# Prayforhanluo/HiCHap_master

Measured on AMD Instinct MI355X. Metric: ICE iterations/sec on 10 kb whole-genome matrix (also nnz*iters/sec), higher is better.
Workload: dtype f64; 1 GPU; hg19-10kb-diploid-wholegenome; n_bins=607282, nnz_upper=4998527599, resolution_bp=10000, parallelism=single GPU, entries_stored=9997055198, slots_u32=160483740, slots_u16=3356357472, payload_bytes=14884946704, tiles=89023, units=89007, hbm_bytes_matrix=15833045375

## Files before the change

hichap_master_amd/_lib.py:

```python
from __future__ import annotations

import ctypes as C
import os

_HERE = os.path.dirname(os.path.abspath(__file__))
LIB_PATH = os.environ.get("HH_LIB") or os.path.join(_HERE, "libhichap_hip.so")

HH_OK = 0


class HipLibraryError(RuntimeError):

    def __init__(self, code, msg):
        super().__init__(f"[hh rc={code}] {msg}")
        self.code = code


class MatrixInfo(C.Structure):
    _fields_ = [(n, C.c_int64) for n in (
        "n_bins", "row_lo", "row_hi", "nnz_upper", "n_entries", "n_slots", "n_tiles",
        "n_units", "n_wide", "device_bytes", "n_slots_narrow", "payload_bytes")] + [
        (n, C.c_int32) for n in ("n_chroms", "ignore_diags", "cis_only", "device", "band_w", "n_units_flat")] + [
        ("n_band", C.c_int64), ("payload_bytes_flat", C.c_int64)] + [
        (n, C.c_int32) for n in ("band_w4", "upper")]
# ... 7 lines not shown
        ("comp_block", C.c_int32), ("ignore_diags", C.c_int32), ("cis_only", C.c_int32),
        ("pad_", C.c_int32), ("seed", C.c_uint64)]


class IceOpts(C.Structure):
    _fields_ = [
        ("mad_max", C.c_int32), ("min_nnz", C.c_int32), ("min_count", C.c_double),
        ("tol", C.c_double), ("max_iters", C.c_int32), ("rescale_marginals", C.c_int32),
        ("check_every", C.c_int32), ("pad_", C.c_int32)]


P = C.c_void_p
I32, I64, F64 = C.c_int32, C.c_int64, C.c_double
PI32, PI64, PF64 = C.POINTER(C.c_int32), C.POINTER(C.c_int64), C.POINTER(C.c_double)

SIGNATURES = {
    "hh_last_error": (C.c_char_p, []),
    "hh_version": (C.c_int, []),
    "hh_device_count": (C.c_int, [PI32]),
    "hh_set_device": (C.c_int, [I32]),
    "hh_synchronize": (C.c_int, [P]),
    "hh_device_copy": (C.c_int, [P, P, I64, P]),
    "hh_tune": (C.c_int, [C.c_char_p, I64]),
    "hh_tune_get": (C.c_int, [C.c_char_p, PI64]),
    "hh_ktime_enable": (C.c_int, [I32]),
    "hh_ktime_query": (C.c_int, [C.c_char_p, P, P]),
    "hh_ktime_reset": (C.c_int, []),
    "hh_matrix_from_pixels": (C.c_int, [P, P, P, I64, I64, P, I32, I32, I32, I64, I64, P, C.POINTER(P)]),
    "hh_matrix_from_pixels_device": (C.c_int, [P, P, P, I64, I64, P, I32, I32, I32, I64, I64, P, C.POINTER(P)]),
    "hh_matrix_free": (C.c_int, [P]),
    "hh_matrix_get_info": (C.c_int, [P, C.POINTER(MatrixInfo)]),
    "hh_matrix_export_upper": (C.c_int, [P, P, P, P, PI64]),
    "hh_synth_count": (C.c_int, [C.POINTER(SynthParams), P, P, P]),
    "hh_synth_build": (C.c_int, [C.POINTER(SynthParams), I64, I64, P, C.POINTER(P)]),
    "hh_synth_dense": (C.c_int, [P, I32, P, P]),
    "hh_synth_pixels": (C.c_int, [C.POINTER(SynthParams), I32, P, C.POINTER(P)]),
    "hh_pixels_get": (C.c_int, [P, P, P, P, PI64]),
    "hh_pixels_free": (C.c_int, [P]),
    "hh_ice_balance": (C.c_int, [P, C.POINTER(IceOpts), P, P, P, P, P, PF64, P]),
    "hh_ice_create": (C.c_int, [P, C.POINTER(IceOpts), C.POINTER(P)]),
    "hh_ice_free": (C.c_int, [P]),
    "hh_ice_n_groups": (C.c_int, [P, PI32]),
    "hh_ice_marg_local": (C.c_int, [P, I32, P, P]),
    "hh_ice_set_marg": (C.c_int, [P, P, I32, I64, P, P]),
    "hh_ice_filter_nnz": (C.c_int, [P, P]),
    "hh_ice_filter_count_mad": (C.c_int, [P, P]),
    "hh_ice_update": (C.c_int, [P, P]),
    "hh_ice_active_groups": (C.c_int, [P, PI32, P]),
    "hh_ice_iterations_done": (C.c_int, [P, PI32]),
    "hh_ice_run": (C.c_int, [P, I32, P]),
    "hh_ice_finalize": (C.c_int, [P, P, P, P, P, P, P]),
    "hh_ice_last_sweep_timing": (C.c_int, [P, PF64, PI32, PF64]),
    "hh_ice_swept_bytes": (C.c_int, [P, PI64]),
    "hh_ice_get_bias": (C.c_int, [P, P, P]),
    "hh_ice_set_bias": (C.c_int, [P, P, P]),
    "hh_ice_uband_fallbacks": (C.c_int, [P, PI64, P]),
    "hh_ice_uband_skipped": (C.c_int, [P, PI64, PI64]),
    "hh_sweep_trace": (C.c_int, [P, I64, PI64]),
    "hh_matrix_stream_probe": (C.c_int, [P, I32, PF64, I32]),
    "hh_comm_unique_id": (C.c_int, [P]),
    "hh_comm_init": (C.c_int, [P, I32, I32, C.POINTER(P)]),
    "hh_comm_free": (C.c_int, [P]),
    "hh_comm_allgather": (C.c_int, [P, I64, P, P, P]),
    "hh_comm_reduce_scatter": (C.c_int, [P, I64, P, P, P]),
    "hh_ice_set_column_exchange": (C.c_int, [P, I32, I32, P, P, P, P, P]),
    "hh_ice_balance_sharded": (C.c_int, [P, C.POINTER(IceOpts), I32, I32, P, P, P, P, P, P, P, P, PF64, P]),
    "hh_ice_balance_cis_local": (C.c_int, [P, C.POINTER(IceOpts), I32, I64, P, P, P, P, P, P, P, PF64, P]),
    "hh_ice_filters_sharded": (C.c_int, [P, I32, P, P, P, P]),
    "hh_ice_run_sharded": (C.c_int, [P, I32, P, P, P, I32, P]),
    "hh_dense_rowstats": (C.c_int, [P, I32, I64, P, P, P, P, I32, P]),
    "hh_dense_symvc": (C.c_int, [P, I32, I64, P, P, F64, F64, P, I32, P]),
    "hh_twostep": (C.c_int, [P, P, P, I64, P, P, P, P, I32, P]),
    "hh_twostep_batch": (C.c_int, [I32, P, P, P, P, P, P, P, P, I32, P]),
    "hh_dense_from_cells": (C.c_int, [P, P, P, I64, I64, I64, I32, I32, P, P]),
    "hh_dense_upper_count": (C.c_int, [P, I64, PI64, P]),
    "hh_dense_upper_write": (C.c_int, [P, I64, P, P, P, P]),
    "hh_comp_create": (C.c_int, [P, I64, I32, P, C.POINTER(P)]),
    "hh_comp_free": (C.c_int, [P]),
    "hh_comp_colnnz": (C.c_int, [P, P, P]),
    "hh_comp_diag_sums": (C.c_int, [P, P, P, P]),
    "hh_comp_sliding_oe": (C.c_int, [P, P, I32, P]),
    "hh_comp_get_sliding_oe": (C.c_int, [P, P, P]),
    "hh_comp_correlation": (C.c_int, [P, P, P, I64, P]),
    "hh_comp_get_cor": (C.c_int, [P, P, P]),
    "hh_comp_set_cor": (C.c_int, [P, P, P]),
    "hh_gap_scan": (C.c_int, [P, I64, I32, I32, P, I32, P]),
    "hh_di_scan": (C.c_int, [P, I64, I32, P, P, I32, P, I32, P]),
    "hh_band_from_pixels": (C.c_int, [P, P, P, I64, P, I64, I64, I64, I32, P, I32, P]),
    "hh_tad_scan_pixels": (C.c_int, [P, P, P, I64, P, I64, I64, I64, I32, P, I32, P, P, I32, P]),
    "hh_insulation_scan": (C.c_int, [P, I64, I32, P, P, I32, I32, P, P, I32, P]),
    "hh_insulation_pixels": (C.c_int, [P, P, P, I64, P, I64, I64, I64, P, P, I32, I32, P, P, I32, P]),
    "hh_viterbi_gmm": (C.c_int, [P, I64, I32, I32, P, P, P, P, P, P, P]),
    "hh_hmm_bw_create": (C.c_int, [P, P, I64, I32, I32, P, C.POINTER(P)]),
    "hh_hmm_bw_free": (C.c_int, [P]),
    "hh_hmm_bw_step": (C.c_int, [P, P, P, P, P, P, F64, PF64]),
    "hh_hmm_bw_train": (C.c_int, [P, P, P, P, P, P, I32, F64, F64, PI32, P, PI32]),
    "hh_hmm_bw_last_step_ms": (C.c_int, [P, PF64]),
    "hh_comp_pca": (C.c_int, [P, I32, F64, I32, P, P, P, P]),
    "hh_comp_select_stats": (C.c_int, [P, P, I32, F64, P, P]),
    "hh_comp_pca_status": (C.c_int, [P, PI32, PI32, PI32, PI32]),
    "hh_sym_topk": (C.c_int, [P, I32, I32, P, P]),
    "hh_binner_create": (C.c_int, [I32, C.c_char_p, P, I32, I32, C.POINTER(P)]),
    "hh_binner_free": (C.c_int, [P]),
    "hh_binner_add_target": (C.c_int, [P, I32, I32, P, P, I64, PI32]),
    "hh_binner_feed": (C.c_int, [P, C.c_char_p, I64, P, I64, P]),
    "hh_binner_add_impute_target": (C.c_int, [P, I32, I32, P, P, I64, P, I32, I64, F64, PI32]),
# ... 130 lines not shown
```

hichap_master_amd/csrc/ice.hip:

```cpp
#include <algorithm>
#include <chrono>
#include <functional>
#include <cmath>
#include <limits>

#include "ice_internal.hpp"

namespace hh {
constexpr int kThreads = 256;

constexpr int kSweepThreads = 512;
constexpr int kSweepWaves = kSweepThreads / 64;
constexpr int kFlatU = 8;
static_assert(kFlatU == kFlatIlvU, "k_sweep_flatw walks the interleaved layout's runs");

__device__ __forceinline__ double lds_b(const double* bl, uint32_t byteoff) {
    return *reinterpret_cast<const double*>(reinterpret_cast<const char*>(bl) + byteoff);
}

__device__ __forceinline__ void tile_dot(const uint4 v, const double* __restrict__ bl, double& a0, double& a1) {
    const uint32_t w[4] = {v.x, v.y, v.z, v.w};
    double x[4];
#pragma unroll
    for (int i = 0; i < 4; ++i) x[i] = lds_b(bl, w[i] & 0xFFFFu);
// ... 2314 lines not shown

using namespace hh;

namespace hh {
constexpr int kFuseMaxTiles = 128;
}

struct hh_ice {
    hh_matrix* m = nullptr;
    hh_ice_opts o{};
    int64_t n = 0, nloc = 0;
    int32_t G = 1;
    std::vector<int64_t> glo, ghi;
    int32_t n_tiles = 0;
    DBuf<int32_t> tile_lo, tile_hi, tile_group, group_tile_ptr, blk_tile_ptr;
    DBuf<double> bias, marg, part, tile_cnt, tile_sum, tile_sq, g_cnt, g_sum;
    DBuf<unsigned> counter;
    bool stats_fresh = false;
    DBuf<double> bpart;
    int32_t nch = 0;
    int32_t nchu = 0;
    DBuf<double> upart;
    DBuf<uint32_t> ub_tasks[2];
    int64_t ub_ntasks[2] = {0, 0}, ub_bytes[2] = {0, 0}, ub_waves_all = 0, ub_waves_dead = 0;
    DBuf<unsigned long long> ub_fallbacks;
    DBuf<uint8_t> halo8, halo4;
    int64_t halo_lo = 0, ub_glo = 0, ub_ghi = 0;
    DBuf<uint8_t> active;
    DBuf<double> g_var, g_mean;
    DBuf<int32_t> g_iters;
    DBuf<uint8_t> g_empty;
    DBuf<long long> rank_rows;
    std::vector<int64_t> h_rank_rows;
    DBuf<unsigned long long> colpart, colacc, bmax, bfix;
    DBuf<double> fix;
    double rmax = 1.0;
    bool rmax_global = false;
    int32_t cx_world = 1, cx_rank = 0;
    int64_t cx_maxlen = 0;
    std::vector<int64_t> cx_rr;
    DBuf<long long> cx_rr_dev;
    hh_reduce_fn cx_fn = nullptr;
    void* cx_user = nullptr;
    hh_allgather_fn cx_ag = nullptr;
    void* cx_ag_user = nullptr;
    DBuf<unsigned long long> cx_send, cx_recv, cx_all;
    int32_t iters_done = 0;
    PinnedBuf<uint8_t> h_active;
    std::vector<hipEvent_t> ev;
    double sweep_ms = 0.0, iter_ms = 0.0;
    int32_t sweep_launches = 0;
    hipStream_t side = nullptr, side2 = nullptr;
    hipEvent_t fork = nullptr, join = nullptr, join2 = nullptr;
    ~hh_ice() {
        for (auto e : ev) (void)hipEventDestroy(e);
        if (join2) (void)hipEventDestroy(join2);
        if (side2) (void)hipStreamDestroy(side2);
        if (fork) (void)hipEventDestroy(fork);
        if (join) (void)hipEventDestroy(join);
        if (side) (void)hipStreamDestroy(side);
    }
    bool full() const { return m->row_lo == 0 && m->row_hi == m->n_bins; }
    TileArgs ta() {
        return TileArgs{tile_lo.p, tile_hi.p, tile_group.p, group_tile_ptr.p, blk_tile_ptr.p, tile_cnt.p,
                        tile_sum.p, tile_sq.p, g_cnt.p, g_sum.p, counter.p};
    }
    bool small_stats() const { return hh::g_fuse_stats == 1 || (hh::g_fuse_stats < 0 && n_tiles <= hh::kFuseMaxTiles); }
    uint8_t* act() { return active.p + (iters_done & 1) * G; }
    uint8_t* nxt() { return active.p + (1 - (iters_done & 1)) * G; }
};

namespace hh {

constexpr int64_t kConcUbMinBytes = 1LL << 30;
constexpr int64_t kUbandMinBytes = 128LL << 20;
constexpr int64_t kSingleMaxBytes = 1LL << 30;

using FlatwKernel = void (*)(TileDev, const uint8_t*, const double*, long long, double*);
template <int PIPE>
static FlatwKernel flatw_by_waves(int nw) {
    switch (nw) {
        case 8: return k_sweep_flatw<kFlatU, PIPE, 8, false>;
        case 10: return k_sweep_flatw<kFlatU, PIPE, 10, false>;
        case 11: return k_sweep_flatw<kFlatU, PIPE, 11, false>;
    }
    return nullptr;
}
static FlatwKernel flatw_kernel(int pipe, int nw) {
    switch (pipe) {
        case 0: return flatw_by_waves<0>(nw);
        case 2: return flatw_by_waves<2>(nw);
        case 3: return flatw_by_waves<3>(nw);
    }
    return nullptr;
}

template <bool UP>
static void launch_sweep(const hh_matrix* m, const TileDev& T, const uint8_t* act, const double* b, double* part,
                            hipStream_t s, hipStream_t s_tiled, int which) {
    const int n_tiled = (int)(m->n_units - m->n_units_flat), n_flat = (int)m->n_units_flat;
    auto tiled = [&] {
        if (!n_tiled) return;
        HH_KTIME("k_sweep_tiled", s_tiled);
        auto kern = k_sweep_tiled<UP, 0>;
        if constexpr (!UP) {
            if (g_tiled_pf == 1) kern = k_sweep_tiled<UP, 1>;
            if (g_tiled_pf == 2) kern = k_sweep_tiled<UP, 2>;
        }
// ... 209 lines not shown
                    : rows == 128 ? k_sweep_bands<128, true>
                                  : k_sweep_bands<256, false>;
        hipLaunchKernelGGL(kern, dim3(rb, (unsigned)nc), dim3(kBandThreads), 0, s, L, (long long)S->nloc,
                           (long long)m->row_lo, (long long)m->n_bins, S->act(), m->row_group.p, S->bias.p,
                           S->bpart.p);
        HIP_CHECK(hipGetLastError());
    };
    if (g_band_fused) {
        launch(segs, ch);
    } else {
        for (int k = 0; k < segs.n; ++k) {
            BandSegs one{};
            one.s[0] = segs.s[k];
            one.n = 1;
            for (int y = 0; y < segs.s[k].nc; ++y) one.ord[y] = (uint8_t)(segs.s[k].ch + y);
            launch(one, segs.s[k].nc);
        }
    }
}

static void sweep_single(hh_ice* S, hipStream_t s) {
    const hh_matrix* m = S->m;
    BandSegs segs;
    const int ch = (S->nch && S->nloc && !S->nchu) ? band_segs(m, segs) : (segs = BandSegs{}, 0);
    const int band_rb = (int)((S->nloc + 63) / 64);
    const int n_tiled = (int)(m->n_units - m->n_units_flat), n_flat = (int)m->n_units_flat;
    const long long n_band = ch ? (long long)band_rb * ch : 0;
    const long long grid = n_tiled + n_band + n_flat;
    if (S->nchu && S->nloc) sweep_uband(S, s);
    if (!grid) return;
    HH_REQUIRE(grid < (1LL << 31), "sweep grid too large for one launch");
    unsigned long long* trace = grid <= g_trace_cap ? g_trace : nullptr;
    if (trace) g_trace_n = grid;
    auto kern = k_sweep_all<kFlatU, false>;
    if constexpr (kUpperBuild) {
        if (m->upper && S->colpart.p) kern = k_sweep_all<kFlatU, true>;
    }
    hipLaunchKernelGGL(kern, dim3((unsigned)grid), dim3(kSweepThreads), 0, s, tdev(S), S->act(), n_tiled,
                       (int)n_band, segs, band_rb, (long long)S->nloc, (long long)m->row_lo, m->row_group.p,
                       S->bias.p, (long long)m->n_bins, S->part.p, S->bpart.p, trace);
    HIP_CHECK(hipGetLastError());
}

static void ensure_side_streams(hh_ice* S) {
    if (S->side) return;
    int cur = 0;
    HIP_CHECK(hipGetDevice(&cur));
    if (cur != S->m->device) HIP_CHECK(hipSetDevice(S->m->device));
    HIP_CHECK(hipStreamCreateWithFlags(&S->side, hipStreamNonBlocking));
    HIP_CHECK(hipEventCreateWithFlags(&S->fork, hipEventDisableTiming));
    HIP_CHECK(hipEventCreateWithFlags(&S->join, hipEventDisableTiming));
    HIP_CHECK(hipStreamCreateWithFlags(&S->side2, hipStreamNonBlocking));
    HIP_CHECK(hipEventCreateWithFlags(&S->join2, hipEventDisableTiming));
    if (cur != S->m->device) HIP_CHECK(hipSetDevice(cur));
}

static void marg_weighted(hh_ice* S, double* out, hipStream_t s, bool timed, int slot) {
    hh_matrix* m = S->m;
    const bool up = m->upper && S->colpart.p;
    const bool shard_x = up && S->cx_world > 1;
    HH_REQUIRE(!shard_x || S->rmax_global,
               "upper-triangle tiles on a shard: run the filters on the gathered marginals first (global scale)");
    if (timed) HIP_CHECK(hipEventRecord(S->ev[2 * slot], s));
    if (up)
        hipLaunchKernelGGL(k_fixscale, dim3(nblocks(std::max<int64_t>(S->n, 1), 256)), dim3(256), 0, s, S->bmax.p,
                           S->iters_done & 1, S->rmax, S->fix.p, S->bias.p, (long long)S->n, S->bfix.p);
    const TileDev T = tdev(S);
    {
        HH_KTIME(timed ? nullptr : "ice_sweep", s);
        const int64_t bytes = 4 * m->n_slots + 2 * m->n_slots_narrow + (int64_t)m->band.n + (int64_t)m->band4.n;
        const bool conc = g_band_concurrent && (S->nch || S->nchu) && S->nloc && m->n_units &&
                          (bytes >= g_conc_min_bytes || (S->nchu && bytes >= kConcUbMinBytes));
        const bool single = !(up && m->n_fgroups) && !m->flat_perm &&
                            (g_sweep_single == 1 || (g_sweep_single == -1 && bytes < kSingleMaxBytes));
        if (single) {
            sweep_single(S, s);
        } else if (conc) {
            ensure_side_streams(S);
            HIP_CHECK(hipEventRecord(S->fork, s));
            HIP_CHECK(hipStreamWaitEvent(S->side, S->fork, 0));
            if (g_split_tiles) HIP_CHECK(hipStreamWaitEvent(S->side2, S->fork, 0));
            if (g_conc_order == 1) {
                sweep(m, T, S->act(), S->bias.p, S->part.p, s, s, 2);
                sweep_band(S, S->side);
                sweep(m, T, S->act(), S->bias.p, S->part.p, s, g_split_tiles ? S->side2 : s, 1);
            } else if (g_conc_order == 2) {
                sweep(m, T, S->act(), S->bias.p, S->part.p, s, s, 2);
                sweep(m, T, S->act(), S->bias.p, S->part.p, s, g_split_tiles ? S->side2 : s, 1);
                sweep_band(S, S->side);
            } else {
                sweep_band(S, S->side);
                sweep(m, T, S->act(), S->bias.p, S->part.p, s, g_split_tiles ? S->side2 : s);
            }
            HIP_CHECK(hipEventRecord(S->join, S->side));
            if (g_split_tiles) {
                HIP_CHECK(hipEventRecord(S->join2, S->side2));
                HIP_CHECK(hipStreamWaitEvent(s, S->join2, 0));
            }
            HIP_CHECK(hipStreamWaitEvent(s, S->join, 0));
        } else {
            sweep(m, T, S->act(), S->bias.p, S->part.p, s);
            sweep_band(S, s);
        }
        if (up && S->n > 0) {
            hipLaunchKernelGGL(k_colsum, dim3(nblocks(S->n, 256)), dim3(256), 0, s, S->colpart.p, m->jslot_ptr.p,
                               m->jslot.p, 0LL, (long long)S->n, S->colacc.p);
            HIP_CHECK(hipGetLastError());
        }
    }
    if (timed) HIP_CHECK(hipEventRecord(S->ev[2 * slot + 1], s));
    const unsigned long long* col_own = up ? S->colacc.p + m->row_lo : nullptr;
    if (shard_x) {
        const long long tot = (long long)S->cx_world * S->cx_maxlen;
        hipLaunchKernelGGL(k_colpad, dim3(nblocks(tot, kThreads)), dim3(kThreads), 0, s, S->colacc.p, S->cx_world,
                           (long long)S->cx_maxlen, S->cx_rr_dev.p, S->cx_send.p);
        HIP_CHECK(hipGetLastError());
        int rc = 0;
        if (S->cx_fn) {
            rc = S->cx_fn(reinterpret_cast<const int64_t*>(S->cx_send.p), S->cx_maxlen,
                          reinterpret_cast<int64_t*>(S->cx_recv.p), S->cx_user, s);
        } else {
            rc = S->cx_ag(reinterpret_cast<const double*>(S->cx_send.p), tot, reinterpret_cast<double*>(S->cx_all.p),
                          S->cx_ag_user, s);
            if (!rc)
                hipLaunchKernelGGL(k_colgather, dim3(nblocks(S->cx_maxlen, kThreads)), dim3(kThreads), 0, s,
                                   S->cx_all.p, S->cx_world, (long long)S->cx_maxlen, S->cx_rank, S->cx_recv.p);
        }
        if (rc) HH_THROW(rc < 0 ? rc : HH_ERR_HIP, std::string("column exchange failed: ") + hh_last_error());
        col_own = S->cx_recv.p;
    }
// ... 47 lines not shown
}

}

static void filter_count_mad(hh_ice* S, hipStream_t s,
                             const std::function<std::vector<double>(const std::vector<double>&)>& gather) {
    if (S->o.min_count != 0.0)
        hipLaunchKernelGGL(k_filter_lt, dim3(nblocks(S->n, kThreads)), dim3(kThreads), 0, s, S->marg.p,
                           (long long)S->n, S->o.min_count, S->bias.p);
    HIP_CHECK(hipGetLastError());
    if (S->o.mad_max <= 0) return;
    std::vector<double> marg(S->n), bias(S->n);
    {
        PinnedDown dl;
        dl.add(S->marg.p, marg.data(), (size_t)S->n);
        dl.add(S->bias.p, bias.data(), (size_t)S->n);
        dl.run(s);
    }
    const auto& off = S->m->chrom_offsets;
    std::vector<double> pos;
    for (int c = 0; c < S->m->n_chroms; ++c) {
        pos.clear();
        for (int64_t i = off[c]; i < off[c + 1]; ++i)
            if (marg[i] > 0) pos.push_back(marg[i]);
        const double med = np_median(pos);
        for (int64_t i = off[c]; i < off[c + 1]; ++i) marg[i] = marg[i] / med;
    }
    const std::vector<double> all = gather ? gather(marg) : marg;
    std::vector<double> logm;
    for (double x : all)
        if (x > 0) logm.push_back(std::log(x));
    const double med = np_median(logm);
    std::vector<double> dev(logm.size());
    for (size_t k = 0; k < logm.size(); ++k) dev[k] = std::fabs(logm[k] - med);
    const double cutoff = std::exp(med - S->o.mad_max * np_median(dev));
    for (int64_t i = 0; i < S->n; ++i)
        if (marg[i] < cutoff) bias[i] = 0.0;
    upload_pinned_sync(S->bias.p, bias.data(), (size_t)S->n, s);
}

extern "C" {

int hh_ice_create(hh_matrix* m, const hh_ice_opts* o, hh_ice** out) {
    return guard([&] {
        HH_REQUIRE(m && out, "null");
        check_opts(o);
        HIP_CHECK(hipSetDevice(m->device));
        auto S = std::make_unique<hh_ice>();
        S->m = m;
        S->o = *o;
        if (S->o.check_every <= 0) S->o.check_every = 8;
        S->n = m->n_bins;
        S->nloc = m->nloc();
        if (m->cis_only) {
            S->G = m->n_chroms;
            for (int c = 0; c < m->n_chroms; ++c) {
                S->glo.push_back(m->chrom_offsets[c]);
                S->ghi.push_back(m->chrom_offsets[c + 1]);
            }
        } else {
            S->G = 1;
            S->glo = {0};
            S->ghi = {m->n_bins};
        }
        std::vector<int32_t> tlo, thi, tg, gtp(S->G + 1, 0);
        for (int g = 0; g < S->G; ++g) {
            gtp[g] = (int32_t)tlo.size();
            for (int64_t b = S->glo[g]; b < S->ghi[g];) {
                const int64_t e = std::min<int64_t>((b / kR + 1) * kR, S->ghi[g]);
                tlo.push_back((int32_t)b);
                thi.push_back((int32_t)e);
                tg.push_back(g);
                b = e;
            }
        }
        gtp[S->G] = (int32_t)tlo.size();
        S->n_tiles = (int32_t)tlo.size();
        const int64_t nblk = (S->n + kR - 1) / kR;
        std::vector<int32_t> btp(nblk + 1, 0);
        for (size_t t = 0, B = 0; B <= (size_t)nblk; ++B) {
            while (t < tlo.size() && tlo[t] < (int64_t)B * kR) ++t;
            btp[B] = (int32_t)t;
        }
        hipStream_t s = 0;
        S->tile_lo = to_device(tlo, s);
        S->tile_hi = to_device(thi, s);
        S->tile_group = to_device(tg, s);
        S->group_tile_ptr = to_device(gtp, s);
        S->blk_tile_ptr = to_device(btp, s);
        S->g_cnt.alloc(S->G);
        S->g_sum.alloc(S->G);
        S->counter.alloc(2);
        S->counter.zero(s);
        S->bias.alloc(S->n);
        std::vector<double> ones(S->n, 1.0);
        upload_pinned_sync(S->bias.p, ones.data(), (size_t)S->n, s);
        S->marg.alloc(S->n);
        S->marg.zero(s);
        S->part.alloc(std::max<int64_t>(m->n_part, 1));
        S->nch = m->band_w > 0 ? (int32_t)((band_stride(m->band_w) + kBandChunk - 1) / kBandChunk) : 0;
        if (m->band_w4 > m->band_w)
            S->nch += 2 * (int32_t)((band4_seg(m->band_w, m->band_w4) + kBandChunk - 1) / kBandChunk);
        const int64_t band_all = m->n_bins * ((m->band_w > 0 ? band_stride(m->band_w) : 0) +
                                              (m->band_w4 > m->band_w ? band4_stride(m->band_w, m->band_w4) : 0));
        if (S->nch && (g_uband == 2 || (g_uband == 1 && band_all >= kUbandMinBytes))) {
            const long long dmax = std::max<long long>(m->band_w, m->band_w4);
// ... 160 lines not shown
        hipStream_t s = as_stream(stream);
        HIP_CHECK(hipMemcpyAsync(S->h_active.p, S->act(), S->G, hipMemcpyDeviceToHost, s));
        HIP_CHECK(hipStreamSynchronize(s));
        int a = 0;
        for (int g = 0; g < S->G; ++g) a += S->h_active.p[g] ? 1 : 0;
        *n_active = a;
    });
}

int hh_ice_iterations_done(const hh_ice* S, int32_t* iters) {
    return guard([&] { HH_REQUIRE(S && iters, "null"); *iters = S->iters_done; });
}

int hh_ice_run(hh_ice* S, int32_t n, void* stream) {
    return guard([&] {
        HH_REQUIRE(S && n >= 0, "bad arguments");
        HH_REQUIRE(S->full(), "hh_ice_run needs a matrix holding every row (use the sharded API)");
        hipStream_t s = as_stream(stream);
        const size_t need = 2 * (size_t)n + 2;
        while (S->ev.size() < need) {
            hipEvent_t e;
            HIP_CHECK(hipEventCreate(&e));
            S->ev.push_back(e);
        }
        HIP_CHECK(hipEventRecord(S->ev[2 * n], s));
        const bool ev = g_iter_events != 0;
        for (int k = 0; k < n; ++k) {
            marg_weighted(S, S->marg.p, s, ev, k);
            update(S, s);
        }
        HIP_CHECK(hipEventRecord(S->ev[2 * n + 1], s));
        HIP_CHECK(hipStreamSynchronize(s));
        double tot = 0.0;
        for (int k = 0; ev && k < n; ++k) {
            float ms = 0.f;
            HIP_CHECK(hipEventElapsedTime(&ms, S->ev[2 * k], S->ev[2 * k + 1]));
            tot += ms;
        }
        float all = 0.f;
        HIP_CHECK(hipEventElapsedTime(&all, S->ev[2 * n], S->ev[2 * n + 1]));
        S->sweep_ms = tot;
        S->iter_ms = all;
        S->sweep_launches = n;
    });
}

int hh_ice_last_sweep_timing(const hh_ice* S, double* sweep_ms_total, int32_t* sweep_launches,
                             double* iter_ms_total) {
    return guard([&] {
        HH_REQUIRE(S, "null");
        if (sweep_ms_total) *sweep_ms_total = S->sweep_ms;
        if (sweep_launches) *sweep_launches = S->sweep_launches;
        if (iter_ms_total) *iter_ms_total = S->iter_ms;
    });
}

int hh_ice_set_column_exchange(hh_ice* S, int32_t world, int32_t rank, const int64_t* rank_rows, hh_reduce_fn reduce,
                               void* reduce_user, hh_allgather_fn allgather, void* allgather_user) {
    return guard([&] {
        HH_REQUIRE(S && world >= 1 && rank_rows && rank >= -1 && rank < world, "bad arguments");
        HH_REQUIRE(world == 1 || reduce || allgather || (S->cx_fn && S->cx_world == world),
                   "a reduce or all-gather function is required for world > 1");
        std::vector<int64_t> rr(rank_rows, rank_rows + world + 1);
        HH_REQUIRE(rr[0] == 0 && rr[world] == S->n, "rank_rows must span [0, n_bins]");
        int64_t maxlen = 1;
        for (int k = 0; k < world; ++k) {
            HH_REQUIRE(rr[k] <= rr[k + 1], "rank_rows not monotone");
            maxlen = std::max<int64_t>(maxlen, rr[k + 1] - rr[k]);
        }
        if (rank < 0) {
            for (int k = 0; k < world && rank < 0; ++k)
                if (rr[k] == S->m->row_lo && rr[k + 1] == S->m->row_hi) rank = k;
            HH_REQUIRE(rank >= 0, "the matrix shard is none of rank_rows' ranges");
        }
        HH_REQUIRE(rr[rank] == S->m->row_lo && rr[rank + 1] == S->m->row_hi,
                   "the matrix shard does not hold rank_rows[rank] .. rank_rows[rank + 1]");
        if (!reduce && S->cx_fn && S->cx_world == world) {
            reduce = S->cx_fn;
            reduce_user = S->cx_user;
        }
        S->cx_world = world;
        S->cx_rank = rank;
        S->cx_maxlen = maxlen;
        S->cx_fn = reduce;
        S->cx_user = reduce_user;
        S->cx_ag = allgather;
        S->cx_ag_user = allgather_user;
        if (rr != S->cx_rr) {
            S->cx_rr = rr;
            std::vector<long long> ll(rr.begin(), rr.end());
            S->cx_rr_dev = to_device(ll, 0);
            HIP_CHECK(hipStreamSynchronize(0));
        }
        if (world > 1 && S->m->upper) {
            S->cx_send.alloc((size_t)world * maxlen);
            S->cx_recv.alloc((size_t)maxlen);
            if (!reduce) S->cx_all.alloc((size_t)world * world * maxlen);
        }
    });
}

int hh_ice_get_bias(const hh_ice* S, double* bias, void* stream) {
    return guard([&] {
        HH_REQUIRE(S && bias, "null");
        hipStream_t s = as_stream(stream);
        S->bias.download(bias, S->n, s);
// ... 276 lines not shown
```

hichap_master_amd/csrc/ice_internal.hpp:

```cpp
#pragma once

#include "hh_common.hpp"

namespace hh {

constexpr int kR = 512;
#ifndef HH_KWBITS
#define HH_KWBITS 13
#endif
constexpr int kWBits = HH_KWBITS;
constexpr bool kUpperBuild = HH_KWBITS <= 12;
constexpr int kW = 1 << kWBits;
constexpr uint32_t kColMask = kW - 1;
constexpr uint32_t kCntMax = 65535u;
inline int64_t g_unit_entries = 0;
constexpr int64_t kMaxBins = (int64_t)1 << 30;

constexpr uint32_t kNarrowMax = 7;

constexpr int kBandChunk = 2048;
constexpr int kBandMaxW = 16384;
constexpr uint32_t kBandMaxCnt = 255u;
constexpr double kBandDensity = 0.5;
inline int64_t g_band_w = -1;
// ... 193 lines not shown
    }
    hh::TileDev dev(unsigned long long* colpart = nullptr, const double* fix = nullptr,
                    const unsigned long long* bfix = nullptr) const {
        return hh::TileDev{pay.p, payn.p, tile_J.p, tile_ent.p, tile_rp.p, tile_entn.p, tile_rpn.p, u_tlo.p,
                           u_thi.p, u_rb.p, u_rlo.p, u_rhi.p, u_slot.p, u_glo.p, u_ghi.p, blk_unit_ptr.p,
                           u_order.p, tile_perm.p, tile_band.p, tile_fw.p, tile_frec.p,
                           reinterpret_cast<const uint4*>(frec.p), u_whole.p, fg_ptr.p, fg_unit.p, fg_desc.p,
                           hh::g_flat_defer, upper && colpart ? 1 : 0, (long long)row_lo, u_cslot.p, fg_cslot.p,
                           colpart, fix, bfix};
    }
};

namespace hh {
inline std::vector<uint16_t> bin_groups(const hh_matrix& m) {
    std::vector<uint16_t> g(m.n_bins, 0);
    if (m.cis_only)
        for (int c = 0; c < m.n_chroms; ++c)
            for (int64_t b = m.chrom_offsets[c]; b < m.chrom_offsets[c + 1]; ++b) g[b] = (uint16_t)c;
    return g;
}
void upload_plan(const TilePlan& P, hh_matrix& m, hipStream_t s);

constexpr int kFlatIlvU = 8;
__host__ __device__ inline uint32_t flat_ilv_cnt(uint32_t m, int k) {
    return m > (uint32_t)k ? (m - (uint32_t)k + kFlatIlvU - 1) / kFlatIlvU : 0u;
}
__host__ __device__ inline uint32_t flat_ilv_pos(uint32_t m, uint32_t i) {
    const int k = (int)(i % kFlatIlvU);
    uint32_t b = 0;
    for (int j = 0; j < k; ++j) b += flat_ilv_cnt(m, j);
    return b + i / kFlatIlvU;
}
void finalize_flat_layout(hh_matrix& m, hipStream_t s);
void narrow_payload_plain(const hh_matrix& m, DBuf<uint16_t>& out, hipStream_t s);
void dev_sort_u64(DBuf<unsigned long long>& keys, int64_t n, int bits, hipStream_t s, int lo_bit = 0);
int64_t dev_sort_cells_by_col(const int32_t* r, const int32_t* c, const uint32_t* v, int64_t nnz, int fmt, int ib,
                              int cbits, DBuf<unsigned long long>& keys, hipStream_t s);
void dev_excl_scan_i64(const long long* in, long long* out, long long n, unsigned long long* total_dev, hipStream_t s);
bool build_from_host_pixels_on_device(const int64_t* bin1, const int64_t* bin2, const double* count, int64_t nnz,
                                      int64_t n_bins, const int64_t* chrom_offsets, int32_t n_chroms,
                                      int32_t ignore_diags, int32_t cis_only, int64_t row_lo, int64_t row_hi,
                                      hipStream_t s, hh_matrix** out);
inline int64_t g_host_build = 0;
inline int64_t g_build_debug = 0;

inline int g_flatw_waves = 11;
inline int g_flatw_waves_up = 8;
inline int g_flatw_pipe = 3;
inline int g_tiled_pf = 1;
inline int g_band_concurrent = 1;
inline int g_split_tiles = 1;
inline int g_conc_order = 1;
inline int64_t g_conc_min_bytes = 8LL << 30;
inline int g_band_rows = 0;
inline int g_band_fused = 1;
inline int g_uband = 1;
inline int g_ub_skip = 1;
inline int g_ub_xcd = 1;
inline int g_ub_fast = 1;
inline int g_sweep_single = -1;
inline int g_iter_events = 1;
inline int g_fuse_stats = -1;
inline unsigned long long* g_trace = nullptr;
inline int64_t g_trace_cap = 0, g_trace_n = 0;
}
```

hichap_master_amd/csrc/tune.hip:

```cpp
#include <climits>

#include "ice_internal.hpp"

namespace hh {
namespace {

struct Knob {
    const char* name;
    int* vi;
    int64_t* vl;
    int64_t lo, hi, step;
    int n_also;
    int64_t also[5];
    const char* doc;
};

Knob range(const char* name, int* v, int64_t lo, int64_t hi, const char* doc) {
    return Knob{name, v, nullptr, lo, hi, 0, 0, {}, doc};
}
Knob range(const char* name, int64_t* v, int64_t lo, int64_t hi, const char* doc) {
    return Knob{name, nullptr, v, lo, hi, 0, 0, {}, doc};
}
Knob set_of(const char* name, int* v, std::initializer_list<int64_t> set, const char* doc) {
    Knob k{name, v, nullptr, 1, 0, 0, 0, {}, doc};
    for (int64_t x : set) k.also[k.n_also++] = x;
    return k;
}

const Knob kKnobs[] = {
    Knob{"band_w", nullptr, &g_band_w, 0, kBandMaxW, 16, 1, {-1}, "uint8 band half-width: -1 auto, 0 off, else forced"},
    range("band4", &g_band4, 0, 1, "nibble band beyond the uint8 band"),
    range("band_cis", &g_band_cis, 0, 1, "the bands hold cis pixels only (0: by diagonal and count alone)"),
    range("flat_max", &g_flat_max, 0, 255, "longest row (uint4) of a flat tile segment, 0: no flat tiles"),
    range("flat_cols", &g_flat_cols, -1, 1, "flat tiles swept by column group: -1 auto, 0, 1"),
    range("flat_group", &g_flat_group, 0, 256, "flat tiles per column group, 0: auto (11 .. 44)"),
    Knob{"unit_entries", nullptr, &g_unit_entries, 4096, 1 << 24, 0, 1, {0}, "payload words per work unit, 0: auto"},
    range("upper_tiles", &g_upper_tiles, -1, 1, "upper-triangle tiles: -1 auto, 0, 1 (the 4096-column build only)"),
    range("host_build", &g_host_build, 0, 1, "1: the host builder for every pixel table"),
    range("build_debug", &g_build_debug, 0, 9, "build and balance phase times on stderr"),
    set_of("flatw_pipe", &g_flatw_pipe, {0, 2, 3}, "k_sweep_flatw: 0 no prefetch, 2 masked prefetch, 3 raw prefetch"),
    set_of("flatw_waves", &g_flatw_waves, {8, 10, 11}, "waves per k_sweep_flatw block"),
    set_of("flatw_waves_up", &g_flatw_waves_up, {8, 11}, "the same for the column-side kernel"),
    range("flat_defer", &g_flat_defer, 0, 1, "k_sweep_flat merges a tile's sums after the next tile's barrier"),
    range("tiled_pf", &g_tiled_pf, 0, 2, "k_sweep_tiled: 0 plain loops, 1 pipelined loads, 2 and rows reduced in turn"),
    set_of("band_rows", &g_band_rows, {0, 64, 128, 256}, "rows per band block, 0: auto"),
    range("band_fused", &g_band_fused, 0, 1, "the band segments in one launch"),
    range("band_concurrent", &g_band_concurrent, 0, 1, "the band sweep on a side stream"),
    range("split_tiles", &g_split_tiles, 0, 1, "with band_concurrent: the tiled kernel on a second side stream"),
    range("conc_order", &g_conc_order, 0, 2, "three-stream launch order"),
    range("conc_min_bytes", &g_conc_min_bytes, 0, INT64_MAX, "payload from which the sweep forks into streams"),
    range("uband", &g_uband, 0, 2, "upper-band sweep: 0 off, 1 auto, 2 always"),
    range("ub_skip", &g_ub_skip, 0, 1, "upper-band sweep leaves out the dead rectangles"),
    range("ub_xcd", &g_ub_xcd, 0, 1, "upper-band blocks in contiguous ranges per XCD"),
    range("ub_fast", &g_ub_fast, 0, 1, "upper-band walk on exponent-zero operands"),
    range("sweep_single", &g_sweep_single, -1, 1, "the whole sweep in one launch: -1 auto, 0, 1"),
    range("iter_events", &g_iter_events, 0, 1, "hh_ice_run: HIP events around every sweep"),
    range("fuse_stats", &g_fuse_stats, -1, 2, "stats mode: -1 auto, 0 unfused, 1 small, 2 big (changes results)"),
    Knob{"sweep_trace", nullptr, nullptr, 0, INT32_MAX, 0, 0, {}, "block capacity of the one-launch sweep's timeline"},
    range("pca_method", &g_pca_method, 0, 1, "0 block subspace iteration, 1 block Krylov"),
    range("pca_p", &g_pca_p, 2, 8, "Cor products per Krylov cycle"),
    range("pca_coop", &g_pca_coop, 0, 1, "Krylov orthogonalisation in one launch per product"),
    range("pca_debug", &g_pca_debug, 0, 9, "per-cycle trace on stderr"),
    range("syrk_split", &g_syrk_split, -1, 64, "Cov K splits: -1 auto, 0 never, n forced (changes results)"),
    range("cor_sym", &g_cor_sym, 0, 3, "Krylov Cor products on the upper triangle: 0 full, 1, 2, 3"),
    set_of("ortho_tpb", &g_ortho_tpb, {0, 1, 2, 4, 8}, "k_ortho rows per block / 64, 0: auto"),
    range("ortho_min_tpb", &g_ortho_min_tpb, 1, 2, "the automatic choice's smallest ortho_tpb"),
    range("ortho_lowsync", &g_ortho_lowsync, 0, 1, "k_ortho's Full mode as low-synch CGS2"),
    range("ortho_grid_cap", &g_ortho_grid_cap, 0, 64, "a lower cap on k_ortho's grid, 0: none"),
    range("ortho_abort_test", &g_ortho_abort_test, 0, 2, "act as if k_ortho's barrier timed out (tests)"),
    Knob{"symvc_rows", &g_symvc_rows, nullptr, 16, 1024, 16, 0, {}, "rows per k_ts_gemv block"},
    range("symvc_out", &g_symvc_out, 0, 1, "pass 3 with one LDS tile"),
    range("symvc_stream", &g_symvc_stream, 0, 1, "passes 1-2 as row-streaming GEMVs"),
    range("twostep_devglue", &g_twostep_devglue, 0, 1, "gap / alpha glue on the device"),
    Knob{"twostep_budget_mb", nullptr, nullptr, 0, INT64_MAX >> 20, 0, 0, {}, "hh_twostep_batch workspace, 0: free HBM"},
    range("parse_ablate", &g_parse_ablate, 0, 3, "pair parser timing ablations (wrong results while set)"),
    range("rank_lds_buckets", &g_rank_lds_buckets, 0, 8192, "hh_diag_rank_pixels: LDS buckets per block"),
    range("coarsen_tile", &g_coarsen_tile, 64, HH_COARSEN_TILE, "coarse columns per work item"),
    range("saddle_diag_tile", &g_saddle_diag_tile, 64, HH_SADDLE_DIAG_TILE, "diagonals per wave of the expected sums"),
    range("pileup_chunk", &g_pileup_chunk, 1, HH_PILEUP_CHUNK, "features per chunk of the pileup sums (changes results)"),
    Knob{"scc_rows", &g_scc_rows, nullptr, 4, 32, 4, 1, {0}, "rows per work item of the stratum moments, 0: from h (changes results)"},
    range("trans_trips", &g_trans_trips, 1, HH_TRANS_MAX_TRIPS, "trips of 64 pixels per span of the trans block sums (changes results)"),
    range("teig_rows", &g_teig_rows, 1, HH_TEIG_MAX_ROWS, "rows (waves) per block of the trans operator's product"),
};

const Knob* find(const std::string& key) {
    for (const Knob& k : kKnobs)
        if (key == k.name) return &k;
    HH_THROW(HH_ERR_ARG, "unknown tuning key " + key);
}

bool legal(const Knob& k, int64_t v) {
    for (int i = 0; i < k.n_also; ++i)
        if (v == k.also[i]) return true;
    return v >= k.lo && v <= k.hi && (k.step == 0 || v % k.step == 0);
}

std::string allowed(const Knob& k) {
    std::string s = std::string(k.name) + " = ";
    auto num = [](int64_t x) { return x == INT64_MAX ? std::string("2^63 - 1") : std::to_string(x); };
    const char* sep = "";
    if (k.n_also) {
        s += "{";
        for (int i = 0; i < k.n_also; ++i, sep = ", ") s += sep + num(k.also[i]);
// ... 55 lines not shown
```

hichap_master_amd/ice.py:

```python
from __future__ import annotations

import ctypes as C
from dataclasses import asdict, dataclass

import numpy as np

from . import _lib
from ._lib import IceOpts, MatrixInfo, SynthParams, call, ptr


@dataclass
class IceOptions:
    ignore_diags: int = 1
    cis_only: bool = False
    mad_max: int = 5
    min_nnz: int = 10
    min_count: float = 0
    tol: float = 1e-5
    max_iters: int = 200
    rescale_marginals: bool = True
    check_every: int = 8

    def c_opts(self) -> IceOpts:
        return IceOpts(int(self.mad_max), int(self.min_nnz), float(self.min_count), float(self.tol),
# ... 202 lines not shown
        call("hh_ice_create", m.handle, C.byref(opts.c_opts()), C.byref(h))
        self._h = h
        g = C.c_int32(0)
        call("hh_ice_n_groups", h, C.byref(g))
        self.n_groups = g.value

    def marg_local(self, mode, out=None, stream=None):
        call("hh_ice_marg_local", self._h, int(mode), ptr(out), stream)

    def bind_exchange(self, ex):
        if ex.world <= 1:
            return
        self._rs = ex.reduce_callback()
        rr = np.ascontiguousarray(ex.rank_rows, dtype=np.int64)
        call("hh_ice_set_column_exchange", self._h, int(ex.world), -1, ptr(rr), C.cast(self._rs, C.c_void_p),
             None, None, None)

    def set_marg(self, gathered, world, maxlen, rank_rows, stream=None):
        rr = np.ascontiguousarray(rank_rows, dtype=np.int64)
        call("hh_ice_set_marg", self._h, ptr(gathered), int(world), int(maxlen), ptr(rr), stream)

    def filter_nnz(self, stream=None):
        call("hh_ice_filter_nnz", self._h, stream)

    def filter_count_mad(self, stream=None):
        call("hh_ice_filter_count_mad", self._h, stream)

    def update(self, stream=None):
        call("hh_ice_update", self._h, stream)

    def active_groups(self, stream=None) -> int:
        n = C.c_int32(0)
        call("hh_ice_active_groups", self._h, C.byref(n), stream)
        return n.value

    def iterations_done(self) -> int:
        n = C.c_int32(0)
        call("hh_ice_iterations_done", self._h, C.byref(n))
        return n.value

    def run(self, n, stream=None):
        call("hh_ice_run", self._h, int(n), stream)

    def last_timing(self):
        ms, k, it = C.c_double(0), C.c_int32(0), C.c_double(0)
        call("hh_ice_last_sweep_timing", self._h, C.byref(ms), C.byref(k), C.byref(it))
        return ms.value, k.value, it.value

    def swept_bytes(self):
        b = C.c_int64(0)
        call("hh_ice_swept_bytes", self._h, C.byref(b))
        return b.value

    def bias(self, stream=None):
        b = np.empty(int(self.m.info()["n_bins"]))
        call("hh_ice_get_bias", self._h, ptr(b), stream)
        return b

    def set_bias(self, b, stream=None):
        b = np.ascontiguousarray(b, dtype=np.float64)
        if b.shape != (int(self.m.info()["n_bins"]),):
            raise ValueError("set_bias: one bias per bin")
        call("hh_ice_set_bias", self._h, ptr(b), stream)

    def uband_fallbacks(self, stream=None) -> int:
        n = C.c_int64(0)
        call("hh_ice_uband_fallbacks", self._h, C.byref(n), stream)
        return n.value

    def uband_skipped(self):
        dead, tot = C.c_int64(0), C.c_int64(0)
        call("hh_ice_uband_skipped", self._h, C.byref(dead), C.byref(tot))
        return dead.value, tot.value

    def finalize(self, stream=None):
        n = int(self.m.info()["n_bins"])
        G = self.n_groups
        w = np.empty(n)
        scale, var = np.empty(G), np.empty(G)
        iters, conv = np.empty(G, np.int32), np.empty(G, np.int32)
        call("hh_ice_finalize", self._h, ptr(w), ptr(scale), ptr(var), ptr(iters), ptr(conv), stream)
        return w, _stats(self.opts, scale, var, iters, conv, self.m.info()["cis_only"])

    def close(self):
        if self._h:
            call("hh_ice_free", self._h)
            self._h = None

    def __del__(self):
        try:
            self.close()
        except Exception:
            pass


__all__ = ["IceOptions", "ContactMatrix", "IceState", "SynthPixels", "DevArray", "balance", "balance_matrix",
           "cooler_balance_cmd", "synth_row_counts", "synth_params", "asdict"]
```

include/hichap_hip.h:

```cpp
#ifndef HICHAP_HIP_H
#define HICHAP_HIP_H

#include <stdint.h>

#ifdef __cplusplus
extern "C" {
#endif

#define HH_OK 0
#define HH_ERR_ARG -1
#define HH_ERR_HIP -2
#define HH_ERR_OOM -3
#define HH_ERR_STATE -4

const char* hh_last_error(void);
int hh_version(void);
int hh_device_count(int32_t* n);
int hh_set_device(int32_t device);
int hh_synchronize(void* stream);
int hh_device_copy(void* dst, const void* src, int64_t bytes, void* stream);
int hh_tune(const char* key, int64_t value);
int hh_tune_get(const char* key, int64_t* value);
int hh_sweep_trace(uint64_t* out, int64_t cap, int64_t* n);
int hh_ktime_enable(int32_t on);
// ... 47 lines not shown
    double comp_strength;
    double vis_sigma;
    double gap_frac;
    double trans_density;
    int32_t comp_block;
    int32_t ignore_diags;
    int32_t cis_only;
    int32_t pad_;
    uint64_t seed;
} hh_synth_params;

int hh_synth_count(const hh_synth_params* p, int32_t* row_work, int64_t* row_nnz_upper,
                   void* stream);
int hh_synth_dense(const hh_synth_params* p, int32_t chrom, double* out, void* stream);
typedef struct hh_pixels hh_pixels;
int hh_synth_pixels(const hh_synth_params* p, int32_t ordered, void* stream, hh_pixels** out);
int hh_pixels_get(const hh_pixels* P, const int32_t** bin1, const int32_t** bin2, const int32_t** count, int64_t* nnz);
int hh_pixels_free(hh_pixels* P);
int hh_synth_build(const hh_synth_params* p, int64_t row_lo, int64_t row_hi, void* stream,
                   hh_matrix** out);

typedef struct {
    int32_t mad_max;
    int32_t min_nnz;
    double min_count;
    double tol;
    int32_t max_iters;
    int32_t rescale_marginals;
    int32_t check_every;
    int32_t pad_;
} hh_ice_opts;

int hh_ice_balance(hh_matrix* m, const hh_ice_opts* o, double* weights, double* scale,
                   double* var, int32_t* iters, int32_t* converged, double* sweep_seconds,
                   void* stream);

typedef struct hh_ice hh_ice;
int hh_ice_create(hh_matrix* m, const hh_ice_opts* o, hh_ice** out);
int hh_ice_free(hh_ice* s);
int hh_ice_n_groups(const hh_ice* s, int32_t* n);
int hh_ice_marg_local(hh_ice* s, int32_t mode, double* marg_local, void* stream);
int hh_ice_set_marg(hh_ice* s, const double* gathered, int32_t world, int64_t maxlen,
                    const int64_t* rank_rows, void* stream);
int hh_ice_filter_nnz(hh_ice* s, void* stream);
int hh_ice_filter_count_mad(hh_ice* s, void* stream);
int hh_ice_update(hh_ice* s, void* stream);
int hh_ice_active_groups(hh_ice* s, int32_t* n_active, void* stream);
int hh_ice_iterations_done(const hh_ice* s, int32_t* iters);
int hh_ice_run(hh_ice* s, int32_t n, void* stream);
int hh_ice_finalize(hh_ice* s, double* weights, double* scale, double* var, int32_t* iters,
                    int32_t* converged, void* stream);
int hh_ice_last_sweep_timing(const hh_ice* s, double* sweep_ms_total, int32_t* sweep_launches,
                             double* iter_ms_total);
int hh_ice_swept_bytes(const hh_ice* s, int64_t* bytes);
int hh_ice_get_bias(const hh_ice* s, double* bias, void* stream);
int hh_ice_set_bias(hh_ice* s, const double* bias, void* stream);
int hh_ice_uband_fallbacks(const hh_ice* s, int64_t* count, void* stream);
int hh_ice_uband_skipped(const hh_ice* s, int64_t* dead_waves, int64_t* all_waves);

typedef int (*hh_allgather_fn)(const double* send, int64_t count, double* recv, void* user, void* stream);
typedef struct hh_comm hh_comm;
int hh_comm_unique_id(uint8_t* id128);
int hh_comm_init(const uint8_t* id128, int32_t world, int32_t rank, hh_comm** out);
int hh_comm_free(hh_comm* c);
int hh_comm_allgather(const double* send, int64_t count, double* recv, void* comm, void* stream);
typedef int (*hh_reduce_fn)(const int64_t* send, int64_t count, int64_t* recv, void* user, void* stream);
int hh_comm_reduce_scatter(const int64_t* send, int64_t count, int64_t* recv, void* comm, void* stream);
int hh_ice_set_column_exchange(hh_ice* s, int32_t world, int32_t rank, const int64_t* rank_rows, hh_reduce_fn reduce,
                               void* reduce_user, hh_allgather_fn allgather, void* allgather_user);
int hh_ice_balance_sharded(hh_matrix* m, const hh_ice_opts* o, int32_t world, int32_t rank, const int64_t* rank_rows,
                           hh_allgather_fn allgather, void* user, double* weights, double* scale, double* var,
                           int32_t* iters, int32_t* converged, double* sweep_seconds, void* stream);
int hh_ice_balance_cis_local(hh_matrix* m, const hh_ice_opts* o, int32_t world, int64_t max_local_bins,
                             hh_allgather_fn allgather, void* user, double* weights, double* scale, double* var,
                             int32_t* iters, int32_t* converged, double* sweep_seconds, void* stream);
int hh_ice_filters_sharded(hh_ice* s, int32_t world, const int64_t* rank_rows, hh_allgather_fn allgather, void* user,
                           void* stream);
int hh_ice_run_sharded(hh_ice* s, int32_t world, const int64_t* rank_rows, hh_allgather_fn allgather, void* user,
                       int32_t n, void* stream);

int hh_dense_rowstats(const void* X, int32_t dtype, int64_t N, const int64_t* lo, const int64_t* hi,
                      double* rowsum, int64_t* zeros, int32_t on_device, void* stream);
int hh_dense_symvc(const void* X, int32_t dtype, int64_t N, const double* alpha, const uint8_t* gap,
                   double exponent, double raw_sum, double* out, int32_t on_device, void* stream);
int hh_dense_from_cells(const int64_t* row, const int64_t* col, const int64_t* count, int64_t nnz, int64_t N,
                        int64_t offset, int32_t symmetric, int32_t on_device, int64_t* out, void* stream);
int hh_dense_upper_count(const double* X, int64_t N, int64_t* nnz, void* stream);
int hh_dense_upper_write(const double* X, int64_t N, int32_t* bin1, int32_t* bin2, double* value, void* stream);
int hh_twostep(const int64_t* TM, const int64_t* MM, const int64_t* PM, int64_t N, double* nor_mm, double* nor_pm,
               uint8_t* gap_m, uint8_t* gap_p, int32_t on_device, void* stream);
int hh_twostep_batch(int32_t n, const int64_t* const* TM, const int64_t* const* MM, const int64_t* const* PM,
                     const int64_t* N, double* const* nor_mm, double* const* nor_pm, uint8_t* gap_m,
                     uint8_t* gap_p, int32_t n_streams, void* stream);

typedef struct hh_gw hh_gw;
int hh_gw_create(const int64_t* t_bin1, const int64_t* t_bin2, const double* t_count, int64_t t_nnz,
                 const int64_t* h_row, const int64_t* h_col, const double* h_count, int64_t h_nnz, int64_t n,
                 const int64_t* chrom_offsets, int32_t n_chroms, void* stream, hh_gw** out);
int hh_gw_create_device(const int32_t* t_bin1, const int32_t* t_bin2, const int32_t* t_count, int64_t t_nnz,
                        const int32_t* h_row, const int32_t* h_col, const int32_t* h_count, int64_t h_nnz, int64_t n,
                        const int64_t* chrom_offsets, int32_t n_chroms, void* stream, hh_gw** out);
int hh_gw_free(hh_gw* g);
int hh_gw_stats(const hh_gw* g, int64_t* t_rowsum, int64_t* t_nnz_row, int64_t* h_blocksum, int64_t* h_total);
int hh_gw_alpha(const hh_gw* g, double* alpha, int32_t* chrom_ok);
int hh_gw_correct(hh_gw* g, const double* alpha, double exponent, int64_t* out_nnz, void* stream);
int hh_gw_correct_count(hh_gw* g, const double* alpha, double exponent, int64_t* out_nnz, void* stream);
// ... 210 lines not shown
```

Before: 384.5 ICE iterations/s.

## Add sweep schedule selector with flat-first phase and CU-based auto choice

```diff
diff --git a/hichap_master_amd/_lib.py b/hichap_master_amd/_lib.py
--- a/hichap_master_amd/_lib.py
+++ b/hichap_master_amd/_lib.py
@@ -83,6 +83,7 @@
     "hh_ice_finalize": (C.c_int, [P, P, P, P, P, P, P]),
     "hh_ice_last_sweep_timing": (C.c_int, [P, PF64, PI32, PF64]),
     "hh_ice_swept_bytes": (C.c_int, [P, PI64]),
+    "hh_ice_sweep_sched": (C.c_int, [P, PI32]),
     "hh_ice_get_bias": (C.c_int, [P, P, P]),
     "hh_ice_set_bias": (C.c_int, [P, P, P]),
     "hh_ice_uband_fallbacks": (C.c_int, [P, PI64, P]),
diff --git a/hichap_master_amd/csrc/ice.hip b/hichap_master_amd/csrc/ice.hip
--- a/hichap_master_amd/csrc/ice.hip
+++ b/hichap_master_amd/csrc/ice.hip
@@ -2390,8 +2390,11 @@
     int32_t sweep_launches = 0;
     hipStream_t side = nullptr, side2 = nullptr;
     hipEvent_t fork = nullptr, join = nullptr, join2 = nullptr;
+    hipEvent_t phase = nullptr;
+    int32_t n_cu = 0;
     ~hh_ice() {
         for (auto e : ev) (void)hipEventDestroy(e);
+        if (phase) (void)hipEventDestroy(phase);
         if (join2) (void)hipEventDestroy(join2);
         if (side2) (void)hipStreamDestroy(side2);
         if (fork) (void)hipEventDestroy(fork);
@@ -2707,7 +2710,29 @@
     HIP_CHECK(hipEventCreateWithFlags(&S->join, hipEventDisableTiming));
     HIP_CHECK(hipStreamCreateWithFlags(&S->side2, hipStreamNonBlocking));
     HIP_CHECK(hipEventCreateWithFlags(&S->join2, hipEventDisableTiming));
+    HIP_CHECK(hipEventCreateWithFlags(&S->phase, hipEventDisableTiming));
     if (cur != S->m->device) HIP_CHECK(hipSetDevice(cur));
+}
+
+static bool band_launches(const hh_ice* S) {
+    if (!S->nloc) return false;
+    if (S->nchu) return S->ub_ntasks[g_ub_skip ? 1 : 0] > 0;
+    return S->nch > 0;
+}
+
+static int sweep_sched(const hh_ice* S) {
+    const hh_matrix* m = S->m;
+    const bool up = m->upper && S->colpart.p;
+    const int64_t bytes = 4 * m->n_slots + 2 * m->n_slots_narrow + (int64_t)m->band.n + (int64_t)m->band4.n;
+    const bool single = !(up && m->n_fgroups) && !m->flat_perm &&
+                        (g_sweep_single == 1 || (g_sweep_single == -1 && bytes < kSingleMaxBytes));
+    if (single) return 3;
+    const bool forks = g_band_concurrent && (bytes >= g_conc_min_bytes || (S->nchu && bytes >= kConcUbMinBytes));
+    if (!forks || g_sweep_sched == 0) return 0;
+    if (g_sweep_sched == 2) return 2;
+    if (!((S->nch || S->nchu) && S->nloc && m->n_units)) return 0;
+    if (g_sweep_sched == 1) return 1;
+    return S->full() && m->n_fgroups >= S->n_cu ? 0 : 1;
 }
 
 static void marg_weighted(hh_ice* S, double* out, hipStream_t s, bool timed, int slot) {
@@ -2723,14 +2748,26 @@
     const TileDev T = tdev(S);
     {
         HH_KTIME(timed ? nullptr : "ice_sweep", s);
-        const int64_t bytes = 4 * m->n_slots + 2 * m->n_slots_narrow + (int64_t)m->band.n + (int64_t)m->band4.n;
-        const bool conc = g_band_concurrent && (S->nch || S->nchu) && S->nloc && m->n_units &&
-                          (bytes >= g_conc_min_bytes || (S->nchu && bytes >= kConcUbMinBytes));
-        const bool single = !(up && m->n_fgroups) && !m->flat_perm &&
-                            (g_sweep_single == 1 || (g_sweep_single == -1 && bytes < kSingleMaxBytes));
-        if (single) {
+        const int sched = sweep_sched(S);
+        if (sched == 3) {
             sweep_single(S, s);
-        } else if (conc) {
+        } else if (sched == 2) {
+            const bool flat = m->n_units_flat > 0, tiled = m->n_units > m->n_units_flat;
+            if (!band_launches(S)) {
+                sweep(m, T, S->act(), S->bias.p, S->part.p, s);
+            } else if (!flat && !tiled) {
+                sweep_band(S, s);
+            } else {
+                ensure_side_streams(S);
+                sweep(m, T, S->act(), S->bias.p, S->part.p, s, s, 2);
+                HIP_CHECK(hipEventRecord(S->phase, s));
+                sweep(m, T, S->act(), S->bias.p, S->part.p, s, s, 1);
+                HIP_CHECK(hipStreamWaitEvent(S->side, S->phase, 0));
+                sweep_band(S, S->side);
+                HIP_CHECK(hipEventRecord(S->join, S->side));
+                HIP_CHECK(hipStreamWaitEvent(s, S->join, 0));
+            }
+        } else if (sched == 1) {
             ensure_side_streams(S);
             HIP_CHECK(hipEventRecord(S->fork, s));
             HIP_CHECK(hipStreamWaitEvent(S->side, S->fork, 0));
@@ -2884,6 +2921,7 @@
         if (S->o.check_every <= 0) S->o.check_every = 8;
         S->n = m->n_bins;
         S->nloc = m->nloc();
+        HIP_CHECK(hipDeviceGetAttribute(&S->n_cu, hipDeviceAttributeMultiprocessorCount, m->device));
         if (m->cis_only) {
             S->G = m->n_chroms;
             for (int c = 0; c < m->n_chroms; ++c) {
@@ -3150,6 +3188,13 @@
         if (sweep_ms_total) *sweep_ms_total = S->sweep_ms;
         if (sweep_launches) *sweep_launches = S->sweep_launches;
         if (iter_ms_total) *iter_ms_total = S->iter_ms;
+    });
+}
+
+int hh_ice_sweep_sched(const hh_ice* S, int32_t* sched) {
+    return guard([&] {
+        HH_REQUIRE(S && sched, "null");
+        *sched = sweep_sched(S);
     });
 }
 
diff --git a/hichap_master_amd/csrc/ice_internal.hpp b/hichap_master_amd/csrc/ice_internal.hpp
--- a/hichap_master_amd/csrc/ice_internal.hpp
+++ b/hichap_master_amd/csrc/ice_internal.hpp
@@ -269,6 +269,7 @@
 inline int g_split_tiles = 1;
 inline int g_conc_order = 1;
 inline int64_t g_conc_min_bytes = 8LL << 30;
+inline int g_sweep_sched = -1;
 inline int g_band_rows = 0;
 inline int g_band_fused = 1;
 inline int g_uband = 1;
diff --git a/hichap_master_amd/csrc/tune.hip b/hichap_master_amd/csrc/tune.hip
--- a/hichap_master_amd/csrc/tune.hip
+++ b/hichap_master_amd/csrc/tune.hip
@@ -49,6 +49,7 @@
     range("split_tiles", &g_split_tiles, 0, 1, "with band_concurrent: the tiled kernel on a second side stream"),
     range("conc_order", &g_conc_order, 0, 2, "three-stream launch order"),
     range("conc_min_bytes", &g_conc_min_bytes, 0, INT64_MAX, "payload from which the sweep forks into streams"),
+    range("sweep_sched", &g_sweep_sched, -1, 2, "sweep schedule: -1 auto, 0 one stream, 1 all concurrent, 2 flat alone then tiled beside band"),
     range("uband", &g_uband, 0, 2, "upper-band sweep: 0 off, 1 auto, 2 always"),
     range("ub_skip", &g_ub_skip, 0, 1, "upper-band sweep leaves out the dead rectangles"),
     range("ub_xcd", &g_ub_xcd, 0, 1, "upper-band blocks in contiguous ranges per XCD"),
diff --git a/hichap_master_amd/ice.py b/hichap_master_amd/ice.py
--- a/hichap_master_amd/ice.py
+++ b/hichap_master_amd/ice.py
@@ -278,6 +278,11 @@
         call("hh_ice_swept_bytes", self._h, C.byref(b))
         return b.value
 
+    def sweep_sched(self) -> int:
+        n = C.c_int32(-1)
+        call("hh_ice_sweep_sched", self._h, C.byref(n))
+        return n.value
+
     def bias(self, stream=None):
         b = np.empty(int(self.m.info()["n_bins"]))
         call("hh_ice_get_bias", self._h, ptr(b), stream)
diff --git a/include/hichap_hip.h b/include/hichap_hip.h
--- a/include/hichap_hip.h
+++ b/include/hichap_hip.h
@@ -123,6 +123,7 @@
                     int32_t* converged, void* stream);
 int hh_ice_last_sweep_timing(const hh_ice* s, double* sweep_ms_total, int32_t* sweep_launches,
                              double* iter_ms_total);
+int hh_ice_sweep_sched(const hh_ice* s, int32_t* sched);
 int hh_ice_swept_bytes(const hh_ice* s, int64_t* bytes);
 int hh_ice_get_bias(const hh_ice* s, double* bias, void* stream);
 int hh_ice_set_bias(hh_ice* s, const double* bias, void* stream);
```

Measured after the change: 397.1 ICE iterations/s (median of 6 runs). 1.03x the previous value.
